# dspcraft/dsc

Measured on AMD Instinct MI355X. Metric: batched 1-D rfft GSamples/s, higher is better.
Workload: dtype f32

## Files before the change

### dsc_amd/csrc/fft_driver.cpp

```cpp
#include "dsc_internal.h"
#include "kernels.h"

#include <cmath>
#include <cstdlib>
#include <cstring>
#include <vector>

static void unit_root(long long k, long long n, long double *c, long double *s) {
    k %= n;
    const long long q = (4 * k) / n;
    const long long r = 4 * k - q * n;
    const long double a = 1.57079632679489661923132169163975144L * (long double) r / (long double) n;
    const long double cr = r == 0 ? 1.0L : cosl(a), sr = r == 0 ? 0.0L : sinl(a);
    switch (q) {
        case 0:  *c = cr;  *s = -sr; break;
        case 1:  *c = -sr; *s = -cr; break;
        case 2:  *c = -cr; *s = sr;  break;
        default: *c = sr;  *s = cr;  break;
    }
}

template<typename T>
static void fill_roots(T *dst, long long count, long long n) {
    for (long long k = 0; k < count; ++k) {
// ... 420 lines not shown
            ctx->last_fft_path = "regs_tiny";
            return;
        }
    }

    static const bool regs_mid_off = getenv("DSC_NO_REGS_MID") != nullptr;
    if (inner == 1 && !regs_mid_off && dsc_fft_regs_small_supports(j.L)) {
        const int x_n = j.x->shape[j.slot];
        const int want = j.mode == DSC_MODE_R2C_PACKED ? 2 * j.L : j.mode == DSC_MODE_C2R_PACKED ? j.L + 1 : j.L;
        const bool full = j.in_len == want && x_n == want;
        if (full || (long long) x_n * 16 * 256 < (1LL << 30)) {
            dsc_launch_fft_regs_mid(j.x->data, j.out->data, n_lines, j.L, j.mode, j.inverse, sp, plan->tw_full, plan->tw_real, j.scale,
                                    full ? -1 : x_n, j.in_len, ctx->stream);
            ctx->last_fft_path = "regs_small";
            return;
        }
    }
    if (inner == 1 && !regs_mid_off && dsc_fft_regs_mid_supports(j.L, j.mode, sp)) {
        const int x_n = j.x->shape[j.slot];
        const int want = j.mode == DSC_MODE_R2C_PACKED ? 2 * j.L : j.mode == DSC_MODE_C2R_PACKED ? j.L + 1 : j.L;
        const bool full = j.in_len == want && x_n == want;
        if (full || (long long) x_n * 16 * 64 < (1LL << 30)) {
            dsc_launch_fft_regs_mid(j.x->data, j.out->data, n_lines, j.L, j.mode, j.inverse, sp, plan->tw_full, plan->tw_real, j.scale,
                                    full ? -1 : x_n, j.in_len, ctx->stream);
            ctx->last_fft_path = "regs_mid";
            return;
        }
    }

    if (j.L <= dsc_fft_lds_max_len(sp)) {
        dsc_fft_lines_args a;
        a.in = j.x->data; a.out = j.out->data;
        a.n_lines = n_lines; a.inner = inner;
        a.lin = lin; a.lout = lout;
        a.L = j.L; a.in_len = j.in_len; a.inverse = j.inverse; a.scale = j.scale;
        a.tw = plan->tw_full; a.tw_real = plan->tw_real; a.tw4_len = 0; a.tw4 = nullptr;
        dsc_launch_fft_lines(a, j.mode, sp, ctx->stream);
        ctx->last_fft_path = "generic_lds";
        return;
    }
    run_four_step(ctx, j, sp, plan);
}

static dsc_tensor *make_out(dsc_ctx *ctx, const dsc_tensor *x, dsc_tensor *out, const int *out_shape, dsc_dtype out_dtype) {
    if (out == nullptr)
        return dsc_new_tensor(ctx, x->n_dim, &out_shape[DSC_MAX_DIMS - x->n_dim], out_dtype, nullptr);
    DSC_ASSERT(out->dtype == out_dtype);
    DSC_ASSERT(out->n_dim == x->n_dim);
    DSC_ASSERT(memcmp(out_shape, out->shape, DSC_MAX_DIMS * sizeof(int)) == 0);
    return out;
}

static dsc_tensor *internal_fft(dsc_ctx *ctx, const dsc_tensor *x, dsc_tensor *out, int n, int axis, bool forward) {
    DSC_ASSERT(x != nullptr);
    dsc_trace_scope trace__(ctx, forward ? "dsc_fft" : "dsc_ifft", "op;fft", x, nullptr, n, axis);
    const int slot = dsc_axis_slot(x, axis);
    DSC_ASSERT(slot >= 0 && slot < DSC_MAX_DIMS);
    const int x_n = x->shape[slot];
    n = n > 0 ? dsc_pow2_n(n) : dsc_pow2_n(x_n);

    int out_shape[DSC_MAX_DIMS];
    for (int i = 0; i < DSC_MAX_DIMS; ++i) out_shape[i] = i != slot ? x->shape[i] : n;
    dsc_dtype out_dtype = x->dtype;
    if (x->dtype == DSC_F32) out_dtype = DSC_C32;
    else if (x->dtype == DSC_F64) out_dtype = DSC_C64;
    out = make_out(ctx, x, out, out_shape, out_dtype);

    fft_job j;
    j.x = x; j.out = out; j.slot = slot;
    j.in_len = x_n < n ? x_n : n;
    j.L = n;
    j.mode = dsc_is_complex(x->dtype) ? DSC_MODE_C2C : DSC_MODE_R2C_CAST;
    j.inverse = !forward;
    j.scale = forward ? 1.0 : 1.0 / (double) n;
    run_job(ctx, j);
    return out;
}

static dsc_tensor *internal_rfft(dsc_ctx *ctx, const dsc_tensor *x, dsc_tensor *out, int n, int axis, bool forward) {
    DSC_ASSERT(x != nullptr);
    dsc_trace_scope trace__(ctx, forward ? "dsc_rfft" : "dsc_irfft", "op;fft", x, nullptr, n, axis);
    const int slot = dsc_axis_slot(x, axis);
    DSC_ASSERT(slot >= 0 && slot < DSC_MAX_DIMS);
    const int x_n = x->shape[slot];

    int out_n, order;
    dsc_dtype out_dtype;
    if (forward) {
        order = (n > 0 ? dsc_pow2_n(n) : dsc_pow2_n(x_n)) >> 1;
        out_n = order + 1;
        if (x->dtype == DSC_F32) out_dtype = DSC_C32;
        else if (x->dtype == DSC_F64) out_dtype = DSC_C64;
        else DSC_LOG_FATAL("RFFT input must be real");
    } else {
        DSC_ASSERT((n > 0 ? n : x_n) > 1);
        order = n > 0 ? dsc_pow2_n(n - 1) : dsc_pow2_n(x_n - 1);
        out_n = order << 1;
        if (x->dtype == DSC_C32) out_dtype = DSC_F32;
        else if (x->dtype == DSC_C64) out_dtype = DSC_F64;
        else DSC_LOG_FATAL("IRFFT input must be complex");
    }
    DSC_ASSERT(order >= 1);

    int out_shape[DSC_MAX_DIMS];
    for (int i = 0; i < DSC_MAX_DIMS; ++i) out_shape[i] = i != slot ? x->shape[i] : out_n;
    out = make_out(ctx, x, out, out_shape, out_dtype);

    fft_job j;
    j.x = x; j.out = out; j.slot = slot;
    j.L = order;
    j.inverse = !forward;
    if (forward) {
        j.mode = DSC_MODE_R2C_PACKED;
        j.in_len = x_n < 2 * order ? x_n : 2 * order;
        j.scale = 1.0;
    } else {
        j.mode = DSC_MODE_C2R_PACKED;
        j.in_len = x_n < order + 1 ? x_n : order + 1;
        j.scale = 2.0 / (double) (order << 1);
    }
    run_job(ctx, j);
    return out;
}

extern "C" dsc_tensor *dsc_fft(dsc_ctx *ctx, const dsc_tensor *x, dsc_tensor *out, int n, int axis) {
    return internal_fft(ctx, x, out, n, axis, true);
}
extern "C" dsc_tensor *dsc_ifft(dsc_ctx *ctx, const dsc_tensor *x, dsc_tensor *out, int n, int axis) {
    return internal_fft(ctx, x, out, n, axis, false);
}
extern "C" dsc_tensor *dsc_rfft(dsc_ctx *ctx, const dsc_tensor *x, dsc_tensor *out, int n, int axis) {
    return internal_rfft(ctx, x, out, n, axis, true);
}
extern "C" dsc_tensor *dsc_irfft(dsc_ctx *ctx, const dsc_tensor *x, dsc_tensor *out, int n, int axis) {
    return internal_rfft(ctx, x, out, n, axis, false);
}

extern "C" dsc_tensor *dsc_filter_fft(dsc_ctx *ctx, const dsc_tensor *s, const dsc_tensor *H, dsc_tensor *out) {
    DSC_ASSERT(s != nullptr && H != nullptr);
    DSC_TRACE_OP(ctx, "op;fft", s, H);
    DSC_ASSERT(dsc_is_complex(H->dtype));
    const int bins = H->shape[DSC_MAX_DIMS - 1];
    DSC_ASSERT(H->ne == bins && bins >= 2);
    const int n = 2 * (bins - 1);
    DSC_ASSERT((n & (n - 1)) == 0);

    const int ls = s->shape[DSC_MAX_DIMS - 1];
    if (s->dtype == DSC_F32 && H->dtype == DSC_C32 && n == 65536) {
        int out_shape[DSC_MAX_DIMS];
        memcpy(out_shape, s->shape, sizeof(out_shape));
        out_shape[DSC_MAX_DIMS - 1] = n;
        out = make_out(ctx, s, out, out_shape, DSC_F32);
        const dsc_fft_plan *plan = dsc_plan_fft(ctx, 32768, DSC_FFT_REAL, DSC_C32);
        dsc_launch_filter64k((const float *) s->data, H->data, (float *) out->data, s->ne / ls, ls, ls < n ? ls : n, plan->tw_aux, ctx->n_cu,
                             ctx->stream);
        ctx->last_fft_path = "filter_64k_regs";
        return out;
    }
    const bool sp_f = s->dtype == DSC_F32 && H->dtype == DSC_C32, dp_f = s->dtype == DSC_F64 && H->dtype == DSC_C64;
    if ((sp_f || dp_f) && dsc_fft_regs_mid_supports(n / 2, DSC_MODE_R2C_PACKED, sp_f) && n / 2 <= 16384 && (long long) ls * 8 * 64 < (1LL << 30)) {
        int out_shape[DSC_MAX_DIMS];
        memcpy(out_shape, s->shape, sizeof(out_shape));
        out_shape[DSC_MAX_DIMS - 1] = n;
        out = make_out(ctx, s, out, out_shape, s->dtype);
        const dsc_fft_plan *plan = dsc_plan_fft(ctx, n / 2, DSC_FFT_REAL, s->dtype);
        dsc_launch_filter_regs_mid(s->data, H->data, out->data, s->ne / ls, n / 2, sp_f, plan->tw_full, plan->tw_real, ls, ls < n ? ls : n,
                                   ctx->stream);
        ctx->last_fft_path = "filter_mid_regs";
        return out;
    }
    dsc_tensor *S = dsc_rfft(ctx, s, nullptr, n, -1);
    dsc_tensor *P = dsc_mul(ctx, S, const_cast<dsc_tensor *>(H), nullptr);
    out = dsc_irfft(ctx, P, out, -1, -1);
    dsc_tensor_free(ctx, S);
    dsc_tensor_free(ctx, P);
    ctx->last_fft_path = "filter_composed";
    return out;
}
```

### dsc_amd/csrc/fft_r2c_64k.hip

```cpp
#include "kernels.h"

#include <hip/hip_runtime.h>

#include <cmath>
#include <cstdlib>
#include <utility>

namespace {

typedef float f2 __attribute__((ext_vector_type(2)));

struct cf { float x, y; };
__device__ __forceinline__ cf operator+(cf a, cf b) { return cf{a.x + b.x, a.y + b.y}; }
__device__ __forceinline__ cf operator-(cf a, cf b) { return cf{a.x - b.x, a.y - b.y}; }
__device__ __forceinline__ cf to_cf(f2 a) { return cf{a.x, a.y}; }
__device__ __forceinline__ f2 to_f2(cf a) { return f2{a.x, a.y}; }

constexpr int kM = 32768;
constexpr int kRowPitch = 34;
constexpr int kPlaneFloats = 1024 * kRowPitch;
constexpr int kLdsBytes = kPlaneFloats * 4 + 1024 * 8;
constexpr int kTabEntries = 1024;

constexpr int kAuxW1024 = 0, kAuxW32768 = 1024, kAuxW65536 = 2048, kAuxEntries = 3072;
// ... 69 lines not shown
    dif_stage<INV, 2>(v, std::make_integer_sequence<int, 16>{});
}


#else
constexpr double kCos64d[17] = {
    1.0, 0.99518472667219688624, 0.98078528040323044913, 0.95694033573220886494,
    0.92387953251128675613, 0.88192126434835502971, 0.83146961230254523708, 0.77301045336273696081,
    0.70710678118654752440, 0.63439328416364549822, 0.55557023301960222474, 0.47139673682599764856,
    0.38268343236508977173, 0.29028467725446236764, 0.19509032201612826785, 0.09801714032956060199,
    0.0};

template<bool INV, int E>
__device__ __forceinline__ void dit_butterfly(cf &a, cf &b) {
    if constexpr (E == 0) {
        const cf u = a + b, d = a - b;
        a = u; b = d;
    } else if constexpr (E == 8) {
        const cf u = INV ? cf{a.x - b.y, a.y + b.x} : cf{a.x + b.y, a.y - b.x};
        const cf d = INV ? cf{a.x + b.y, a.y - b.x} : cf{a.x - b.y, a.y + b.x};
        a = u; b = d;
    } else {
        constexpr double c = E <= 8 ? kCos64d[2 * E] : -kCos64d[32 - 2 * E];
        constexpr double sn = (E <= 8 ? kCos64d[16 - 2 * E] : kCos64d[2 * E - 16]);
        constexpr double s = INV ? sn : -sn;
        if constexpr ((c < 0 ? -c : c) >= sn) {
            constexpr float t = (float) (s / c), cc = (float) c;
            float p, q;
            if constexpr (t == 1.0f) { p = b.x - b.y; q = b.y + b.x; }
            else if constexpr (t == -1.0f) { p = b.x + b.y; q = b.y - b.x; }
            else { p = __builtin_fmaf(-t, b.y, b.x); q = __builtin_fmaf(t, b.x, b.y); }
            const cf u = cf{__builtin_fmaf(cc, p, a.x), __builtin_fmaf(cc, q, a.y)};
            const cf d = cf{__builtin_fmaf(-cc, p, a.x), __builtin_fmaf(-cc, q, a.y)};
            a = u; b = d;
        } else {
            constexpr float r = (float) (c / s), ss = (float) s;
            const float pn = __builtin_fmaf(-r, b.x, b.y);
            const float q = __builtin_fmaf(r, b.y, b.x);
            const cf u = cf{__builtin_fmaf(-ss, pn, a.x), __builtin_fmaf(ss, q, a.y)};
            const cf d = cf{__builtin_fmaf(ss, pn, a.x), __builtin_fmaf(-ss, q, a.y)};
            a = u; b = d;
        }
    }
}

constexpr int brev_bits(int x, int bits) {
    int r = 0;
    for (int i = 0; i < bits; ++i) r |= ((x >> i) & 1) << (bits - 1 - i);
    return r;
}

template<bool INV, int S, int G, int... J>
__device__ __forceinline__ void dit_group(cf (&v)[32], std::integer_sequence<int, J...>) {
    constexpr int H = 32 >> S;
    constexpr int E = brev_bits(G, S - 1) * (16 >> (S - 1));
    (dit_butterfly<INV, E>(v[2 * H * G + J], v[2 * H * G + J + H]), ...);
}

template<bool INV, int S, int... G>
__device__ __forceinline__ void dit_stage(cf (&v)[32], std::integer_sequence<int, G...>) {
    (dit_group<INV, S, G>(v, std::make_integer_sequence<int, (32 >> S)>{}), ...);
}

template<bool INV>
__device__ __forceinline__ void dft32(cf (&v)[32]) {
    dit_stage<INV, 1>(v, std::make_integer_sequence<int, 1>{});
    dit_stage<INV, 2>(v, std::make_integer_sequence<int, 2>{});
    dit_stage<INV, 3>(v, std::make_integer_sequence<int, 4>{});
    dit_stage<INV, 4>(v, std::make_integer_sequence<int, 8>{});
    dit_stage<INV, 5>(v, std::make_integer_sequence<int, 16>{});
}
#endif

typedef unsigned int u2 __attribute__((ext_vector_type(2)));
typedef unsigned int u4 __attribute__((ext_vector_type(4)));
typedef float f4 __attribute__((ext_vector_type(4)));

template<int COMP>
__device__ __forceinline__ void plane_write(float *plane, int wbase, const cf (&v)[32]) {
    int wbase_hi = wbase + 16 * (32 * kRowPitch);
    asm("" : "+v"(wbase_hi));
    float *lo16 = plane + wbase;
    float *hi16 = plane + wbase_hi;
#pragma unroll
    for (int p = 0; p < 32; p += 2) lo16[br5(p) * (32 * kRowPitch)] = COMP == 0 ? v[p].x : v[p].y;
#pragma unroll
    for (int p = 1; p < 32; p += 2) hi16[(br5(p) - 16) * (32 * kRowPitch)] = COMP == 0 ? v[p].x : v[p].y;
}

#ifndef DSC_LDS_SPLIT_READS
#define DSC_LDS_SPLIT_READS 1
#endif
__device__ __forceinline__ f2 lds_read_b64(const f2 *p) {
#if DSC_LDS_SPLIT_READS
    return *(const volatile __attribute__((address_space(3))) f2 *) p;
#else
    return *p;
#endif
}

template<int COMP>
__device__ __forceinline__ void plane_read(const float *plane, int row, cf (&v)[32]) {
    const f2 *r = (const f2 *) (plane + __mul24(row, kRowPitch));
#pragma unroll
    for (int m = 0; m < 16; ++m) {
        const f2 t = lds_read_b64(r + m);
        if (COMP == 0) { v[2 * m].x = t.x; v[2 * m + 1].x = t.y; }
        else           { v[2 * m].y = t.x; v[2 * m + 1].y = t.y; }
    }
}

__device__ __forceinline__ void lds_barrier() {
    __builtin_amdgcn_fence(__ATOMIC_RELEASE, "workgroup", "local");
    __builtin_amdgcn_s_barrier();
    __builtin_amdgcn_fence(__ATOMIC_ACQUIRE, "workgroup", "local");
}

__device__ __forceinline__ float bperm(int byte_addr, float x) {
    return __int_as_float(__builtin_amdgcn_ds_bpermute(byte_addr, __float_as_int(x)));
}

__device__ __forceinline__ int column_of(int wave, int lane) {
    int kp = lane < 32 ? 32 * wave + lane : 1024 - 32 * wave - (63 - lane);
    return kp == 1024 ? 512 : kp;
}

#ifdef DSC_R2C64K_PROBE
#define PROBE_ARGS , int io_on
#define PROBE_NULL , 1
#define IO_ON io_on
#else
#define PROBE_ARGS
#define PROBE_NULL
#define IO_ON 1
#endif

__device__ __forceinline__ int thread_id(int wave_sgpr) {
    int zero;
    asm volatile("v_mov_b32 %0, 0" : "=v"(zero));
    const int lane = __builtin_amdgcn_mbcnt_hi(-1, __builtin_amdgcn_mbcnt_lo(-1, zero));
    return (wave_sgpr << 6) | lane;
}

#ifndef DSC_STREAM_AUX
#define DSC_STREAM_AUX 2
#endif
constexpr int kStream = DSC_STREAM_AUX;
__device__ __forceinline__ cf load_c(__amdgpu_buffer_rsrc_t r, int voff, int soff) {
    return to_cf(__builtin_bit_cast(f2, __builtin_amdgcn_raw_buffer_load_b64(r, voff, soff, kStream)));
}
#ifndef DSC_FILTER_EARLY_LOADS
#define DSC_FILTER_EARLY_LOADS 4
#endif
#ifndef DSC_IRFFT_PIN_PASS3
#define DSC_IRFFT_PIN_PASS3 1
#endif
#ifndef DSC_IRFFT_EARLY_PAIRS
#define DSC_IRFFT_EARLY_PAIRS 4
#endif
#ifndef DSC_IRFFT_LOAD_AUX
#define DSC_IRFFT_LOAD_AUX 0
#endif
__device__ __forceinline__ cf load_c_spec(__amdgpu_buffer_rsrc_t r, int voff, int soff) {
    return to_cf(__builtin_bit_cast(f2, __builtin_amdgcn_raw_buffer_load_b64(r, voff, soff, DSC_IRFFT_LOAD_AUX)));
}
__device__ __forceinline__ cf load_c_cached(__amdgpu_buffer_rsrc_t r, int voff, int soff) {
    return to_cf(__builtin_bit_cast(f2, __builtin_amdgcn_raw_buffer_load_b64(r, voff, soff, 0)));
}
template<int POLICY>
__device__ __forceinline__ void store_c(cf a, __amdgpu_buffer_rsrc_t r, int voff, int soff) {
    __builtin_amdgcn_raw_buffer_store_b64(__builtin_bit_cast(u2, to_f2(a)), r, voff, soff, POLICY);
}

__device__ __forceinline__ void fill_twiddle_table(f2 *T, const f2 *aux) {
    const int t = threadIdx.x;
    T[t] = aux[kAuxW1024 + (t >> 5) * (t & 31)];
    __syncthreads();
}

__device__ __forceinline__ void exchange(float *plane, int wbase, int row, const cf (&src)[32], cf (&dst)[32]) {
    plane_write<0>(plane, wbase, src);
    lds_barrier();
    plane_read<0>(plane, row, dst);
    lds_barrier();
    plane_write<1>(plane, wbase, src);
    lds_barrier();
    plane_read<1>(plane, row, dst);
    lds_barrier();
}

struct no_hook { __device__ __forceinline__ void operator()() const {} };

template<bool INV, typename Hook = no_hook>
__device__ __forceinline__ void three_passes(cf (&v)[32], float *plane, const f2 *T, const f2 *aux, int wave_sgpr,
                                             bool mirrored_in, bool mirrored_out, Hook before_pass3 = Hook{}) {
    dft32<INV>(v);
    cf u[32];
    {
        const int t = thread_id(wave_sgpr);
        const int col = mirrored_in ? column_of(t >> 6, t & 63) : t;
        const int hi = col >> 5;
        const f2 *th = T + hi;
#pragma unroll
        for (int r1 = 1; r1 < 32; ++r1) {
            const cf w = to_cf(th[32 * r1]);
            v[br5(r1)] = INV ? cmul_conj(v[br5(r1)], w) : cmul(v[br5(r1)], w);
        }
        exchange(plane, __mul24(col & 31, kRowPitch) + hi, t, v, u);
    }
    dft32<INV>(u);
    {
        const int t = thread_id(wave_sgpr);
        const int hi = t >> 5, lo = t & 31;
        const cf tw2_base = to_cf(aux[kAuxW32768 + __mul24(hi, lo)]);
        u[0] = INV ? cmul_conj(u[0], tw2_base) : cmul(u[0], tw2_base);
        const f2 *tl = T + lo;
#pragma unroll
        for (int r2 = 1; r2 < 32; ++r2) {
            const cf w = cmul(tw2_base, to_cf(tl[32 * r2]));
            u[br5(r2)] = INV ? cmul_conj(u[br5(r2)], w) : cmul(u[br5(r2)], w);
        }
        const int col_out = mirrored_out ? column_of(t >> 6, t & 63) : t;
        exchange(plane, __mul24(hi, kRowPitch) + lo, col_out, u, v);
    }
    before_pass3();
    dft32<INV>(v);
}

__device__ __forceinline__ void real_pair(cf p, cf q, cf wq, float hs, cf &out_k, cf &out_mk) {
    const cf s = cf{p.x + q.x, p.y - q.y};
    const cf d = cf{p.x - q.x, p.y + q.y};
    const cf wd = cmul(d, wq);
    out_k = cf{hs * s.x + wd.x, hs * s.y + wd.y};
    out_mk = cf{hs * s.x - wd.x, wd.y - hs * s.y};
}

__device__ __forceinline__ int partner_byte_addr(int wave, int lane) {
    return ((wave == 0 && (lane == 63 || lane == 0)) ? lane : 63 - lane) * 4;
}

#ifndef DSC_R2C64K_HELPERS_ONLY
__global__ __launch_bounds__(1024) void rfft64k_kernel(const float *__restrict__ x, f2 *__restrict__ X, int batch,
                                                       const f2 *__restrict__ aux, int in_pitch, int in_len PROBE_ARGS) {
    extern __shared__ __attribute__((aligned(16))) float lds[];
    float *plane = lds;
    f2 *T = (f2 *) (lds + kPlaneFloats);
    fill_twiddle_table(T, aux);

    const int wave_sgpr = __builtin_amdgcn_readfirstlane(threadIdx.x >> 6);

    cf v[32];
    {
        const int row0 = blockIdx.x;
        const __amdgpu_buffer_rsrc_t r0 = __builtin_amdgcn_make_buffer_rsrc(
            (void *) (x + (size_t) row0 * in_pitch), 0, row0 < batch ? in_len * 4 * IO_ON : 0, 0x00020000);
        const int load_off = thread_id(wave_sgpr) * 8;
#pragma unroll
        for (int j1 = 0; j1 < 32; ++j1) v[j1] = load_c(r0, load_off, j1 * 8192);
    }

    for (int row = blockIdx.x; row < batch; row += gridDim.x) {
        const int next_row = row + gridDim.x;
        const __amdgpu_buffer_rsrc_t rnext = __builtin_amdgcn_make_buffer_rsrc(
            (void *) (x + (size_t) next_row * in_pitch), 0, next_row < batch ? in_len * 4 * IO_ON : 0, 0x00020000);
        const __amdgpu_buffer_rsrc_t rout =
            __builtin_amdgcn_make_buffer_rsrc((void *) (X + (size_t) row * (kM + 1)), 0, (kM + 1) * 8 * IO_ON, 0x00020000);

        three_passes<false>(v, plane, T, aux, wave_sgpr, false, true);

        const int t4 = thread_id(wave_sgpr);
        const int lane = t4 & 63, wave = t4 >> 6;
        const int kp = column_of(wave, lane);
        const int partner_addr = partner_byte_addr(wave, lane);
        cf xk[16], xm[16];
        const cf zmid = v[br5(16)];
        if (wave_sgpr == 0) {
#pragma unroll
            for (int r = 16; r < 31; ++r) v[br5(r)] = lane == 0 ? v[br5(r + 1)] : v[br5(r)];
            v[br5(31)] = lane == 0 ? v[br5(0)] : v[br5(31)];
        }
#pragma unroll
        for (int k3 = 0; k3 < 16; ++k3) {
            const int src = 31 - br5(k3);
            xm[k3].x = bperm(partner_addr, v[src].x);
            xm[k3].y = bperm(partner_addr, v[src].y);
        }
        {
            const cf wpost = to_cf(aux[kAuxW65536 + kp]);
            const cf post_base = cf{0.5f * wpost.y, -0.5f * wpost.x};
#pragma unroll
            for (int k3 = 0; k3 < 16; ++k3) {
                const cf c = cf{root64_re(k3), root64_im(k3)};
                const cf w = k3 == 0 ? post_base : cmul(post_base, c);
                real_pair(v[br5(k3)], xm[k3], w, 0.5f, xk[k3], xm[k3]);
            }
        }

        f2 *stage = (f2 *) plane;
        const int skew = (int) ((((size_t) (X + (size_t) row * (kM + 1))) >> 3) & 15);
#pragma unroll
        for (int k3 = 0; k3 < 16; ++k3) stage[kp + 1024 * k3] = to_f2(xk[k3]);
        const cf xk15 = xk[15];
        const int load_off = thread_id(wave_sgpr) * 8;
#pragma unroll
        for (int j1 = 0; j1 < 16; ++j1) v[j1] = load_c(rnext, load_off, j1 * 8192);
        lds_barrier();
// ... 57 lines not shown
            real_pair(v[a], v[16 + a], wq, 0.5f * kScale, v[a], zm[i]);
        }
#pragma unroll
        for (int i = 0; i < 8; ++i) {
            const int a = half * 8 + i;
            v[16 + a].x = bperm(partner_addr, zm[i].x);
            v[16 + a].y = bperm(partner_addr, zm[i].y);
        }
    }
    cf w[32];
#pragma unroll
    for (int r = 0; r < 16; ++r) { w[r] = v[r]; w[16 + r] = v[31 - r]; }
    if (wave == 0) {
#pragma unroll
        for (int r = 31; r > 16; --r) w[r] = lane == 0 ? w[r - 1] : w[r];
        w[16] = lane == 0 ? cf{kScale * y_mid.x, -kScale * y_mid.y} : w[16];
    }
#pragma unroll
    for (int r = 0; r < 32; ++r) v[r] = w[r];
}

template<typename IssueNext>
__device__ __forceinline__ void staged_time_store(cf (&v)[32], float *plane, __amdgpu_buffer_rsrc_t rout, int wave_sgpr,
                                                  IssueNext issue_next) {
    f2 *stage = (f2 *) plane;
    const int t4 = thread_id(wave_sgpr);
#pragma unroll
    for (int p = 0; p < 32; p += 2) stage[t4 + 1024 * br5(p)] = to_f2(v[p]);
    issue_next(true);
    lds_barrier();
#pragma unroll
    for (int m = 0; m < 8; ++m) {
        const int k = 2 * (t4 + 1024 * m);
        const f2 lo2 = lds_read_b64(stage + k), hi2 = lds_read_b64(stage + k + 1);
        const f4 q = f4{lo2.x, lo2.y, hi2.x, hi2.y};
        __builtin_amdgcn_raw_buffer_store_b128(__builtin_bit_cast(u4, q), rout, k * 8, 0, kStream);
        if (m & 1) __builtin_amdgcn_sched_barrier(0);
    }
    lds_barrier();
#pragma unroll
    for (int p = 1; p < 32; p += 2) stage[t4 + 1024 * (br5(p) - 16)] = to_f2(v[p]);
    issue_next(false);
    lds_barrier();
#pragma unroll
    for (int m = 0; m < 8; ++m) {
        const int k = 2 * (t4 + 1024 * m);
        const f2 lo2 = lds_read_b64(stage + k), hi2 = lds_read_b64(stage + k + 1);
        const f4 q = f4{lo2.x, lo2.y, hi2.x, hi2.y};
        __builtin_amdgcn_raw_buffer_store_b128(__builtin_bit_cast(u4, q), rout, (kM / 2 + k) * 8, 0, kStream);
        if (m & 1) __builtin_amdgcn_sched_barrier(0);
    }
    lds_barrier();
}

__device__ __forceinline__ void unzip_rows(cf (&v)[32]) {
    cf nxt[32];
#pragma unroll
    for (int a = 0; a < 16; ++a) { nxt[a] = v[2 * a]; nxt[16 + a] = v[2 * a + 1]; }
#pragma unroll
    for (int a = 0; a < 32; ++a) v[a] = nxt[a];
}

#ifndef DSC_R2C64K_HELPERS_ONLY
__global__ __launch_bounds__(1024) void irfft64k_kernel(const f2 *__restrict__ X, float *__restrict__ x, int batch,
                                                        const f2 *__restrict__ aux, int in_pitch, int in_len PROBE_ARGS) {
    extern __shared__ __attribute__((aligned(16))) float lds[];
    float *plane = lds;
    f2 *T = (f2 *) (lds + kPlaneFloats);
    fill_twiddle_table(T, aux);

    const int wave_sgpr = __builtin_amdgcn_readfirstlane(threadIdx.x >> 6);

    cf v[32];
    cf y_mid = cf{0.f, 0.f};
    {
        const int row0 = blockIdx.x;
        const __amdgpu_buffer_rsrc_t r0 = __builtin_amdgcn_make_buffer_rsrc(
            (void *) (X + (size_t) row0 * in_pitch), 0, row0 < batch ? in_len * 8 * IO_ON : 0, 0x00020000);
        const int t0 = thread_id(wave_sgpr);
        const int c = column_of(t0 >> 6, t0 & 63);
        const int pv = (kM - c - 15 * 1024) * 8;
#pragma unroll
        for (int a = 0; a < 16; ++a) {
            v[a] = load_c_spec(r0, c * 8, a * 8192);
            v[16 + a] = load_c_spec(r0, pv, (15 - a) * 8192);
        }
        if (c == 0) y_mid = load_c_spec(r0, (kM / 2) * 8, 0);
    }

    for (int row = blockIdx.x; row < batch; row += gridDim.x) {
        const int next_row = row + gridDim.x;
        const __amdgpu_buffer_rsrc_t rnext = __builtin_amdgcn_make_buffer_rsrc(
            (void *) (X + (size_t) next_row * in_pitch), 0, next_row < batch ? in_len * 8 * IO_ON : 0, 0x00020000);
        const __amdgpu_buffer_rsrc_t rout =
            __builtin_amdgcn_make_buffer_rsrc((void *) (x + (size_t) row * 65536), 0, 65536 * 4 * IO_ON, 0x00020000);

        inverse_prepass_direct(v, y_mid, aux, wave_sgpr);
        constexpr int kEarly = DSC_IRFFT_EARLY_PAIRS;
        cf early[kEarly > 0 ? 2 * kEarly : 1];
        three_passes<true>(v, plane, T, aux, wave_sgpr, true, false, [&]() {
            if constexpr (kEarly > 0) {
                const int t3 = thread_id(wave_sgpr);
                const int c3 = column_of(t3 >> 6, t3 & 63);
                const int pv3 = (kM - c3 - 15 * 1024) * 8;
#pragma unroll
                for (int a = 0; a < kEarly; ++a) {
                    early[2 * a] = load_c_spec(rnext, c3 * 8, a * 8192);
                    early[2 * a + 1] = load_c_spec(rnext, pv3, (15 - a) * 8192);
                }
            }
        });

#if DSC_IRFFT_PIN_PASS3
#pragma unroll
        for (int p = 0; p < 32; p += 8)
            asm volatile("" : "+v"(v[p].x), "+v"(v[p].y), "+v"(v[p + 1].x), "+v"(v[p + 1].y), "+v"(v[p + 2].x), "+v"(v[p + 2].y), "+v"(v[p + 3].x),
                         "+v"(v[p + 3].y), "+v"(v[p + 4].x), "+v"(v[p + 4].y), "+v"(v[p + 5].x), "+v"(v[p + 5].y), "+v"(v[p + 6].x), "+v"(v[p + 6].y),
                         "+v"(v[p + 7].x), "+v"(v[p + 7].y));
#endif
        const int t4 = thread_id(wave_sgpr);
        const int c = column_of(t4 >> 6, t4 & 63);
        const int pv = (kM - c - 15 * 1024) * 8;
        staged_time_store(v, plane, rout, wave_sgpr, [&](bool first_half) {
            if (first_half) {
                y_mid = cf{0.f, 0.f};
                if (c == 0) y_mid = load_c_spec(rnext, (kM / 2) * 8, 0);
#pragma unroll
                for (int i = 0; i < 8; ++i) {
                    v[2 * i] = load_c_spec(rnext, c * 8, (kEarly + i) * 8192);
                    v[16 + 2 * i] = load_c_spec(rnext, pv, (15 - kEarly - i) * 8192);
                }
            } else {
#pragma unroll
                for (int i = 0; i < 8 - kEarly; ++i) {
                    v[2 * i + 1] = load_c_spec(rnext, c * 8, (kEarly + 8 + i) * 8192);
                    v[17 + 2 * i] = load_c_spec(rnext, pv, (7 - kEarly - i) * 8192);
                }
            }
        });
        {
            cf nxt[32];
#pragma unroll
            for (int a = 0; a < 16; ++a) {
                if (a < kEarly)          { nxt[a] = early[2 * a];             nxt[16 + a] = early[2 * a + 1]; }
                else if (a < kEarly + 8) { nxt[a] = v[2 * (a - kEarly)];      nxt[16 + a] = v[16 + 2 * (a - kEarly)]; }
                else                     { nxt[a] = v[2 * (a - kEarly - 8) + 1]; nxt[16 + a] = v[17 + 2 * (a - kEarly - 8)]; }
            }
#pragma unroll
            for (int a = 0; a < 32; ++a) v[a] = nxt[a];
        }
    }
}

__global__ __launch_bounds__(1024) void filter64k_kernel(const float *__restrict__ x, const f2 *__restrict__ H,
                                                         float *__restrict__ y, int batch, const f2 *__restrict__ aux, int in_pitch,
                                                         int in_len) {
    extern __shared__ __attribute__((aligned(16))) float lds[];
    float *plane = lds;
    f2 *T = (f2 *) (lds + kPlaneFloats);
    fill_twiddle_table(T, aux);

    const int wave_sgpr = __builtin_amdgcn_readfirstlane(threadIdx.x >> 6);
    const __amdgpu_buffer_rsrc_t rh = __builtin_amdgcn_make_buffer_rsrc((void *) H, 0, (kM + 1) * 8, 0x00020000);
    constexpr float kScale = 1.0f / (float) kM;

    cf v[32];
    {
        const int row0 = blockIdx.x;
        const __amdgpu_buffer_rsrc_t r0 = __builtin_amdgcn_make_buffer_rsrc(
            (void *) (x + (size_t) row0 * in_pitch), 0, row0 < batch ? in_len * 4 : 0, 0x00020000);
        const int load_off = thread_id(wave_sgpr) * 8;
#pragma unroll
        for (int j1 = 0; j1 < 32; ++j1) v[j1] = load_c(r0, load_off, j1 * 8192);
    }
    for (int row = blockIdx.x; row < batch; row += gridDim.x) {
        const int next_row = row + gridDim.x;
        const __amdgpu_buffer_rsrc_t rnext = __builtin_amdgcn_make_buffer_rsrc(
            (void *) (x + (size_t) next_row * in_pitch), 0, next_row < batch ? in_len * 4 : 0, 0x00020000);
        const __amdgpu_buffer_rsrc_t rout =
            __builtin_amdgcn_make_buffer_rsrc((void *) (y + (size_t) row * 65536), 0, 65536 * 4, 0x00020000);
        three_passes<false>(v, plane, T, aux, wave_sgpr, false, true);

        {
            const int t1 = thread_id(wave_sgpr);
            const int lane = t1 & 63, wave = t1 >> 6;
            const int c = column_of(wave, lane);
            const int partner_addr = partner_byte_addr(wave, lane);
            const cf wc = to_cf(aux[kAuxW65536 + c]);
            const cf post_base = cf{0.5f * wc.y, -0.5f * wc.x};
            const cf pre_base = cf{0.5f * kScale * wc.y, 0.5f * kScale * wc.x};
            if (wave == 0) {
                const cf zmid = v[br5(16)];
                const cf hmid = load_c_cached(rh, (kM / 2) * 8, 0);
                const cf pmid = cmul(cf{zmid.x, -zmid.y}, hmid);
                v[br5(16)] = lane == 0 ? cf{kScale * pmid.x, -kScale * pmid.y} : v[br5(16)];
            }
            cf park = v[br5(16)];
            if (wave == 0) {
#pragma unroll
                for (int r = 16; r < 31; ++r) v[br5(r)] = lane == 0 ? v[br5(r + 1)] : v[br5(r)];
                v[br5(31)] = lane == 0 ? v[br5(0)] : v[br5(31)];
            }
#pragma unroll
            for (int part = 0; part < 8; ++part) {
                cf q[2], zm[2];
#pragma unroll
                for (int i = 0; i < 2; ++i) {
                    const int a = part * 2 + i;
                    q[i].x = bperm(partner_addr, v[br5(31 - a)].x);
                    q[i].y = bperm(partner_addr, v[br5(31 - a)].y);
                }
#pragma unroll
                for (int i = 0; i < 2; ++i) {
                    const int a = part * 2 + i;
                    const cf w64 = cf{root64_re(a), root64_im(a)};
                    cf xk, xm;
                    real_pair(v[br5(a)], q[i], a == 0 ? post_base : cmul(post_base, w64), 0.5f, xk, xm);
                    const cf hk = load_c_cached(rh, c * 8, a * 8192);
                    const cf hm = load_c_cached(rh, (kM - 15 * 1024 - c) * 8, (15 - a) * 8192);
                    cf pk = cmul(xk, hk), pm = cmul(xm, hm);
                    if (a == 0) {
                        pk.y = (c == 0) ? 0.f : pk.y;
                        pm.y = (c == 0) ? 0.f : pm.y;
                    }
                    const cf w64c = cf{root64_re(a), -root64_im(a)};
                    real_pair(pk, pm, a == 0 ? pre_base : cmul(pre_base, w64c), 0.5f * kScale, v[br5(a)], zm[i]);
                }
#pragma unroll
                for (int i = 0; i < 2; ++i) {
                    const int a = part * 2 + i;
                    v[br5(31 - a)].x = bperm(partner_addr, zm[i].x);
                    v[br5(31 - a)].y = bperm(partner_addr, zm[i].y);
                }
                __builtin_amdgcn_sched_barrier(0);
            }
            if (wave == 0) {
#pragma unroll
                for (int r = 31; r > 16; --r) v[br5(r)] = lane == 0 ? v[br5(r - 1)] : v[br5(r)];
                v[br5(16)] = lane == 0 ? park : v[br5(16)];
            }
        }
        cf z[32];
#pragma unroll
        for (int r = 0; r < 32; ++r) z[r] = v[br5(r)];
        constexpr int kEarlyX = DSC_FILTER_EARLY_LOADS;
        cf early[kEarlyX > 0 ? kEarlyX : 1];
        three_passes<true>(z, plane, T, aux, wave_sgpr, true, false, [&]() {
            if constexpr (kEarlyX > 0) {
                const int off = thread_id(wave_sgpr) * 8;
#pragma unroll
                for (int j1 = 0; j1 < kEarlyX; ++j1) early[j1] = load_c(rnext, off, j1 * 8192);
            }
        });
        {
            const int load_off = thread_id(wave_sgpr) * 8;
            staged_time_store(z, plane, rout, wave_sgpr, [&](bool first_half) {
                if (first_half) {
#pragma unroll
                    for (int i = 0; i < 16; ++i) z[2 * i] = load_c(rnext, load_off, (kEarlyX + i) * 8192);
                } else {
#pragma unroll
                    for (int i = 0; i < 16 - kEarlyX; ++i) z[2 * i + 1] = load_c(rnext, load_off, (kEarlyX + 16 + i) * 8192);
                }
            });
#pragma unroll
            for (int j1 = 0; j1 < 32; ++j1) v[j1] = j1 < kEarlyX ? early[j1] : j1 < kEarlyX + 16 ? z[2 * (j1 - kEarlyX)] : z[2 * (j1 - kEarlyX - 16) + 1];
        }
    }
}

#endif

}

#ifndef DSC_R2C64K_HELPERS_ONLY
size_t dsc_r2c64k_table_bytes() { return (size_t) kAuxEntries * sizeof(float) * 2; }

void dsc_r2c64k_build_tables(void *host_dst) {
    float *o = (float *) host_dst;
    auto put = [&](int at, long long k, long long n) {
        const long double a = -2.0L * 3.14159265358979323846264338327950288L * (long double) k / (long double) n;
        o[2 * at] = (float) cosl(a);
        o[2 * at + 1] = (float) sinl(a);
    };
    for (int m = 0; m < kTabEntries; ++m) {
        put(kAuxW1024 + m, m, 1024);
        put(kAuxW32768 + m, m, 32768);
        put(kAuxW65536 + m, m, 65536);
    }
    o[2 * (kAuxW1024 + 256)] = 0.f;  o[2 * (kAuxW1024 + 256) + 1] = -1.f;
    o[2 * (kAuxW1024 + 512)] = -1.f; o[2 * (kAuxW1024 + 512) + 1] = 0.f;
    o[2 * (kAuxW1024 + 768)] = 0.f;  o[2 * (kAuxW1024 + 768) + 1] = 1.f;
}

void dsc_launch_rfft64k(const float *x, void *X, int batch, int in_pitch, int in_len, const void *aux, int n_cu, hipStream_t stream) {
    if (batch <= 0) return;
    static unsigned long long attr_devices = 0;
    if (dsc_first_use_on_device(attr_devices)) {
        DSC_KERNEL_CHECK(hipFuncSetAttribute((const void *) rfft64k_kernel, hipFuncAttributeMaxDynamicSharedMemorySize, kLdsBytes));
    }
    const int grid = batch < n_cu ? batch : n_cu;
    DSC_LAUNCH(rfft64k_kernel, dim3(grid), dim3(1024), kLdsBytes, stream, x, (f2 *) X, batch, (const f2 *) aux, in_pitch, in_len PROBE_NULL);
}

void dsc_launch_irfft64k(const void *X, float *x, int batch, int in_pitch, int in_len, const void *aux, int n_cu, hipStream_t stream) {
    if (batch <= 0) return;
    static unsigned long long attr_devices = 0;
    if (dsc_first_use_on_device(attr_devices)) {
        DSC_KERNEL_CHECK(hipFuncSetAttribute((const void *) irfft64k_kernel, hipFuncAttributeMaxDynamicSharedMemorySize, kLdsBytes));
    }
    const int grid = batch < n_cu ? batch : n_cu;
    DSC_LAUNCH(irfft64k_kernel, dim3(grid), dim3(1024), kLdsBytes, stream, (const f2 *) X, x, batch, (const f2 *) aux, in_pitch, in_len PROBE_NULL);
}
void dsc_launch_filter64k(const float *s, const void *H, float *y, int batch, int in_pitch, int in_len, const void *aux, int n_cu,
                          hipStream_t stream) {
    if (batch <= 0) return;
    static unsigned long long attr_devices = 0;
    if (dsc_first_use_on_device(attr_devices)) {
        DSC_KERNEL_CHECK(hipFuncSetAttribute((const void *) filter64k_kernel, hipFuncAttributeMaxDynamicSharedMemorySize, kLdsBytes));
    }
    const int grid = batch < n_cu ? batch : n_cu;
    DSC_LAUNCH(filter64k_kernel, dim3(grid), dim3(1024), kLdsBytes, stream, s, (const f2 *) H, y, batch, (const f2 *) aux, in_pitch, in_len);
}
#endif
```

### dsc_amd/csrc/kernels.h

```cpp
#pragma once

#include <hip/hip_runtime.h>
#include <cstddef>
#include <cstdio>
#include <cstdlib>

#define DSC_KERNEL_CHECK(call)                                                                                   \
    do {                                                                                                         \
        hipError_t kerr_ = (call);                                                                               \
        if (kerr_ != hipSuccess) {                                                                               \
            fprintf(stderr, "HIP error %s:%d: %s -> %s\n", __FILE__, __LINE__, #call, hipGetErrorString(kerr_)); \
            exit(EXIT_FAILURE);                                                                                  \
        }                                                                                                        \
    } while (0)
#define DSC_LAUNCH(...)                        \
    do {                                       \
        hipLaunchKernelGGL(__VA_ARGS__);       \
        DSC_KERNEL_CHECK(hipGetLastError());   \
    } while (0)

static inline bool dsc_first_use_on_device(unsigned long long &seen) {
    int dev = 0;
    DSC_KERNEL_CHECK(hipGetDevice(&dev));
    const unsigned long long bit = 1ull << (dev & 63);
    if (seen & bit) return false;
    seen |= bit;
    return true;
}

struct dsc_line_layout {
    long long outer_stride;
    long long inner_stride;
    long long elem_stride;
};

enum dsc_fft_mode {
    DSC_MODE_C2C = 0,
    DSC_MODE_R2C_CAST = 1,
    DSC_MODE_R2C_PACKED = 2,
    DSC_MODE_C2R_PACKED = 3,
};

struct dsc_fft_lines_args {
    const void *in;
    void *out;
    long long n_lines;
    long long inner;
    dsc_line_layout lin, lout;
    int L;
    int in_len;
    int inverse;
    double scale;
    const void *tw;
    const void *tw_real;
    long long tw4_len;
    const void *tw4;
};

int dsc_fft_lds_max_len(bool single_precision);

void dsc_launch_fft_lines(const dsc_fft_lines_args &a, dsc_fft_mode mode, bool single_precision, hipStream_t stream);

void dsc_launch_fft_pack(const void *in, void *work, long long q_first, long long n_lines, long long inner, dsc_line_layout lin,
                         int L, int in_len, dsc_fft_mode mode, bool single_precision, hipStream_t stream);
void dsc_launch_fft_c2r_prepass(const void *in, void *work, long long q_first, long long n_lines, long long inner, dsc_line_layout lin,
                                int L, int in_len, const void *tw_real, bool single_precision, hipStream_t stream);
void dsc_launch_fft_r2c_postpass(const void *work, void *out, long long q_first, long long n_lines, long long inner, dsc_line_layout lout,
                                 int L, const void *tw_real, bool single_precision, hipStream_t stream);
void dsc_launch_fft_unpack(const void *work, void *out, long long q_first, long long n_lines, long long inner, dsc_line_layout lout,
                           int L, double scale, dsc_fft_mode mode, bool single_precision, hipStream_t stream);

size_t dsc_r2c64k_table_bytes();
void   dsc_r2c64k_build_tables(void *host_dst);
void   dsc_launch_rfft64k(const float *x, void *X, int batch, int in_pitch, int in_len, const void *aux, int n_cu, hipStream_t stream);
void   dsc_launch_irfft64k(const void *X, float *x, int batch, int in_pitch, int in_len, const void *aux, int n_cu, hipStream_t stream);
void   dsc_launch_fft32k_c32(const void *z, void *Z, int batch, int in_pitch, int in_len, bool inverse, bool cast, const void *aux, int n_cu,
                             hipStream_t stream);
void   dsc_launch_filter64k(const float *s, const void *H, float *y, int batch, int in_pitch, int in_len, const void *aux, int n_cu,
                            hipStream_t stream);

bool   dsc_fft_regs_cols_supports(int L, dsc_fft_mode mode, bool single_precision);
void   dsc_launch_fft_regs_cols(const void *in, void *out, long long slices, int inner, int L, dsc_fft_mode mode, bool inverse, bool single_precision,
                                const void *tw_full, const void *tw_real, double scale, int in_axis, int in_len, int out_axis, hipStream_t stream);
bool   dsc_fft_cols_4step_split(int n, bool single_precision, int cols, int *n1, int *n2);
void   dsc_launch_rfft_cols_4step(const void *in, void *work, void *out, long long slices, int cc_n, int n1, int n2, bool single_precision,
                                  const void *tw1, const void *tw2, const void *twn, hipStream_t stream);
void   dsc_launch_irfft_cols_4step(const void *in, void *work, void *out, long long slices, int cc_n, int n1, int n2, bool single_precision,
                                   const void *tw1, const void *tw2, const void *twn, double scale, hipStream_t stream);
void   dsc_launch_fft_cols_4step(const void *in, void *work, void *out, long long slices, int inner, int n1, int n2, dsc_fft_mode mode, bool inverse,
                                 bool single_precision, const void *tw1, const void *tw2, const void *twn, double scale, hipStream_t stream);

bool   dsc_fft_two_pass_supports(int L, bool single_precision);
void   dsc_launch_fft_two_pass(const void *in, void *out, long long rows, int L, bool inverse, bool cast, bool single_precision, void *work,
                               const void *tw_full, long long in_pitch, int in_len, hipStream_t stream);
void   dsc_launch_rfft_two_pass(const void *in, void *out, long long rows, int L, bool inverse, bool single_precision, void *work,
                                const void *tw_full, const void *tw_real, long long in_pitch, int in_len, hipStream_t stream);

bool   dsc_fft_fused_l2_supports(int L, bool single_precision, bool real, bool inverse);
size_t dsc_fft_fused_l2_ctl_bytes();
size_t dsc_fft_fused_l2_scratch_bytes(int L, bool single_precision);
bool   dsc_launch_fft_fused_l2(const void *in, void *out, long long rows, int L, bool real, bool inverse, bool cast, bool single_precision, void *scratch,
                               unsigned *host_error, const void *tw_full, const void *tw_real, long long in_pitch, int in_len, hipStream_t stream);

bool dsc_fft_tiny_supports(int L);
void dsc_launch_fft_tiny_cols(const void *in, void *out, long long slices, int inner, int L, dsc_fft_mode mode, bool inverse, bool single_precision,
                              double scale, int in_axis, int in_len, int out_axis, hipStream_t stream);
void dsc_launch_fft_tiny(const void *in, void *out, long long n_lines, int L, dsc_fft_mode mode, bool inverse, bool single_precision, double scale,
                         long long in_pitch, int in_len, hipStream_t stream);

bool dsc_fft_regs_mid_supports(int L, dsc_fft_mode mode, bool single_precision);
bool dsc_fft_regs_small_supports(int L);
void dsc_launch_fft_regs_mid(const void *in, void *out, long long n_lines, int L, dsc_fft_mode mode, bool inverse, bool single_precision,
                             const void *tw_full, const void *tw_real, double scale, long long in_pitch, int in_len, hipStream_t stream);

void dsc_launch_filter_regs_mid(const void *s, const void *H, void *y, long long n_lines, int L, bool single_precision, const void *tw_full,
                                const void *tw_real, long long in_pitch, int in_len, hipStream_t stream);

bool dsc_stft_regs_supports(int n_fft);
void dsc_launch_stft_regs(const void *x, const void *w, void *out, long long n_lines, int n_fft, int T, int n_frames, int hop, int pad,
                          bool reflect, bool single_precision, int x_bytes, const void *tw_full, const void *tw_real, hipStream_t stream);
void dsc_launch_stft_frames(const void *x, const void *w, void *frames, long long q0, long long n_lines, int n_fft, long long T, int n_frames,
                            int hop, int pad, bool reflect, bool single_precision, hipStream_t stream);
void dsc_launch_istft_ola(const void *frames, const void *w, void *y, long long r0, long long rows, int fa, int fpr, int n_fft, int hop,
                          int n_frames, int pad, long long p0, long long p1, int length, bool single_precision, hipStream_t stream);

bool dsc_conv_regs_supports(int n);
void dsc_launch_conv_regs(const void *x, const void *H, void *y, long long n_lines, int n, int T, int n_blocks, int hop, int pad, int D, int T_out,
                          bool single_precision, int x_bytes, int y_bytes, const void *tw_full, const void *tw_real, hipStream_t stream);
void dsc_launch_conv_crop(const void *frames, void *y, long long q0, long long n_lines, int n, int D, int n_blocks, long long T_out,
                          bool single_precision, hipStream_t stream);
void dsc_launch_reverse(const void *in, void *out, int n, bool single_precision, hipStream_t stream);

bool dsc_hilbert_regs_supports(int n);
void dsc_launch_hilbert_regs(const void *x, void *out, long long n_lines, int n, bool envelope, bool single_precision, const void *tw_full,
                             const void *tw_real, long long in_pitch, int in_len, hipStream_t stream);
void dsc_launch_hilbert_response(void *H, int n, bool single_precision, hipStream_t stream);
void dsc_launch_hilbert_zip(const void *x, const void *y, void *out, long long q0, long long n_lines, int n, long long in_pitch, int in_len,
                            bool envelope, bool single_precision, bool y_double, hipStream_t stream);
void dsc_launch_hilbert_widen(const void *x, void *xw, long long q0, long long n_lines, long long in_pitch, int in_len, int wpitch,
                              hipStream_t stream);

bool dsc_fft2_regs_supports(int N0, int N1, dsc_fft_mode mode);
int dsc_fft2_regs_group(int N0, int N1, dsc_fft_mode mode, bool single_precision);
void dsc_launch_fft2_regs(const void *in, void *out, long long n_img, int N0, int N1, int h, int w, dsc_fft_mode mode, bool inverse,
                          bool single_precision, double scale, hipStream_t stream);

void dsc_launch_cast(const void *in, int in_dtype, void *out, int out_dtype, long long ne, hipStream_t stream);

void dsc_launch_unary(const void *in, int in_dtype, void *out, int op, long long ne, hipStream_t stream, double lo = 0, double hi = 0);
void dsc_launch_arange(void *out, int dtype, long long n, hipStream_t stream);

struct dsc_bcast_args {
    int out_shape[4];
    int a_stride[4];
    int b_stride[4];
    long long ne;
    int a_scalar, b_scalar;
    int fast;
    int small_ne;
};
void dsc_launch_binary(const void *a, const void *b, void *out, int dtype, int op, const dsc_bcast_args &g, hipStream_t stream);
bool dsc_launch_binary_mixed(const void *a, int a_dtype, const void *b, int b_dtype, void *out, int op, long long ne, hipStream_t stream);

void dsc_launch_reduce(const void *x, void *out, int dtype, int op, long long outer, int axis_n, long long inner,
                       void *workspace, size_t workspace_bytes, hipStream_t stream);

struct dsc_region {
    int count[4];
    long long stride[4];
    long long base;
    long long ne;
};
void dsc_launch_region_copy(const void *src, void *dst, int elem_bytes, const dsc_region &r, bool scatter, long long dense_ne,
                            hipStream_t stream);

void dsc_launch_transpose_last2(const void *in, void *out, int elem_bytes, long long batch, int rows, int cols, hipStream_t stream);
bool dsc_launch_transpose_moving_last(const void *in, void *out, int elem_bytes, int n_dim, const int *shape, const int *in_stride, const int *perm,
                                      hipStream_t stream);
```

Measured before the change: 652.1.

## Precompute two-term filter coefficients table to fuse r2c/c2r twiddles with H multiply

Adds a small kernel that folds the real-FFT split twiddles, the spectral filter H and the 1/N scale into a per-bin coefficient table (two complex coefficients per bin). The 64k fused filter kernel then loads this table with prefetching and applies the combined operation in a single partner-exchange pass, replacing the separate postpass/multiply/prepass arithmetic. This costs an extra launch and scratch memory per call, plus larger per-bin loads. It is gated by scratch capacity and an environment variable.

```diff
diff --git a/dsc_amd/csrc/fft_driver.cpp b/dsc_amd/csrc/fft_driver.cpp
--- a/dsc_amd/csrc/fft_driver.cpp
+++ b/dsc_amd/csrc/fft_driver.cpp
@@ -596,8 +596,14 @@
         out_shape[DSC_MAX_DIMS - 1] = n;
         out = make_out(ctx, s, out, out_shape, DSC_F32);
         const dsc_fft_plan *plan = dsc_plan_fft(ctx, 32768, DSC_FFT_REAL, DSC_C32);
-        dsc_launch_filter64k((const float *) s->data, H->data, (float *) out->data, s->ne / ls, ls, ls < n ? ls : n, plan->tw_aux, ctx->n_cu,
-                             ctx->stream);
+        const bool no_table = getenv("DSC_FILTER64K_NO_TABLE") != nullptr;
+        void *table = nullptr;
+        if (!no_table && ctx->scratch.capacity() >= dsc_filter64k_table_bytes() + DSC_DEVICE_ALIGN) {
+            ctx->scratch.reset();
+            table = ctx->scratch.alloc(dsc_filter64k_table_bytes());
+        }
+        dsc_launch_filter64k((const float *) s->data, H->data, (float *) out->data, s->ne / ls, ls, ls < n ? ls : n, plan->tw_aux, table,
+                             ctx->n_cu, ctx->stream);
         ctx->last_fft_path = "filter_64k_regs";
         return out;
     }
diff --git a/dsc_amd/csrc/fft_r2c_64k.hip b/dsc_amd/csrc/fft_r2c_64k.hip
--- a/dsc_amd/csrc/fft_r2c_64k.hip
+++ b/dsc_amd/csrc/fft_r2c_64k.hip
@@ -245,6 +245,15 @@
 #ifndef DSC_FILTER_EARLY_LOADS
 #define DSC_FILTER_EARLY_LOADS 4
 #endif
+#ifndef DSC_FILTER_TABLE_AHEAD
+#define DSC_FILTER_TABLE_AHEAD 2
+#endif
+#ifndef DSC_FILTER_TABLE_EARLY
+#define DSC_FILTER_TABLE_EARLY 1
+#endif
+#ifndef DSC_FILTER_TABLE_PIN_PASS3
+#define DSC_FILTER_TABLE_PIN_PASS3 1
+#endif
 #ifndef DSC_IRFFT_PIN_PASS3
 #define DSC_IRFFT_PIN_PASS3 1
 #endif
@@ -608,6 +617,36 @@
     }
 }
 
+constexpr int kCoeffThreads = 256;
+
+__global__ __launch_bounds__(kCoeffThreads) void two_term_coeff64k_kernel(const f2 *__restrict__ H, f4 *__restrict__ D) {
+    const int i = blockIdx.x * kCoeffThreads + threadIdx.x;
+    const int col = i & 1023, slot = i >> 10;
+    const int row = (col == 0 && slot >= 16) ? (slot == 31 ? 16 : slot + 1) : slot;
+    const int k = col + 1024 * row;
+    const f2 hk = H[k], hm = H[kM - k];
+    const double inv = 0.5 / (double) kM;
+    double d1r, d1i, d2r, d2i;
+    if (k == 0) {
+        d1r = (double) hk.x + (double) hm.x; d1i = 0.0;
+        d2r = 0.0;                           d2i = (double) hk.x - (double) hm.x;
+    } else {
+        double sn, cs;
+        sincospi((double) k / (double) kM, &sn, &cs);
+        const double er = (double) hk.x - (double) hm.x, ei = (double) hk.y + (double) hm.y;
+        d1r = (1.0 - sn) * (double) hk.x + (1.0 + sn) * (double) hm.x;
+        d1i = (1.0 - sn) * (double) hk.y - (1.0 + sn) * (double) hm.y;
+        d2r = -cs * ei;
+        d2i = cs * er;
+    }
+    D[i] = f4{(float) (d1r * inv), (float) (d1i * inv), (float) (d2r * inv), (float) (d2i * inv)};
+}
+
+__device__ __forceinline__ cf two_term(cf p, cf q, f4 d) {
+    return cf{d.x * p.x - d.y * p.y + d.z * q.x + d.w * q.y, d.x * p.y + d.y * p.x + d.w * q.x - d.z * q.y};
+}
+
+template<bool TABLE>
 __global__ __launch_bounds__(1024) void filter64k_kernel(const float *__restrict__ x, const f2 *__restrict__ H,
                                                          float *__restrict__ y, int batch, const f2 *__restrict__ aux, int in_pitch,
                                                          int in_len) {
@@ -617,7 +656,7 @@
     fill_twiddle_table(T, aux);
 
     const int wave_sgpr = __builtin_amdgcn_readfirstlane(threadIdx.x >> 6);
-    const __amdgpu_buffer_rsrc_t rh = __builtin_amdgcn_make_buffer_rsrc((void *) H, 0, (kM + 1) * 8, 0x00020000);
+    const __amdgpu_buffer_rsrc_t rh = __builtin_amdgcn_make_buffer_rsrc((void *) H, 0, TABLE ? kM * 16 : (kM + 1) * 8, 0x00020000);
     constexpr float kScale = 1.0f / (float) kM;
 
     cf v[32];
@@ -635,9 +674,72 @@
             (void *) (x + (size_t) next_row * in_pitch), 0, next_row < batch ? in_len * 4 : 0, 0x00020000);
         const __amdgpu_buffer_rsrc_t rout =
             __builtin_amdgcn_make_buffer_rsrc((void *) (y + (size_t) row * 65536), 0, 65536 * 4, 0x00020000);
-        three_passes<false>(v, plane, T, aux, wave_sgpr, false, true);
-
-        {
+        constexpr int kAhead = TABLE ? DSC_FILTER_TABLE_AHEAD : 0;
+        f4 dq[16][2];
+        auto table_offset = [&]() {
+            const int t0 = thread_id(wave_sgpr);
+            return column_of(t0 >> 6, t0 & 63) * 16;
+        };
+        auto load_d = [&](int part, int doff) {
+            dq[part][0] = __builtin_bit_cast(f4, __builtin_amdgcn_raw_buffer_load_b128(rh, doff, part * 16384, 0));
+            dq[part][1] = __builtin_bit_cast(f4, __builtin_amdgcn_raw_buffer_load_b128(rh, doff, (31 - part) * 16384, 0));
+        };
+        three_passes<false>(v, plane, T, aux, wave_sgpr, false, true, [&]() {
+            if constexpr (TABLE && DSC_FILTER_TABLE_EARLY) {
+                const int doff = table_offset();
+#pragma unroll
+                for (int part = 0; part < kAhead; ++part) load_d(part, doff);
+                __builtin_amdgcn_sched_barrier(0);
+            }
+        });
+
+        if constexpr (TABLE) {
+#if DSC_FILTER_TABLE_PIN_PASS3
+#pragma unroll
+            for (int p = 0; p < 32; p += 8)
+                asm volatile("" : "+v"(v[p].x), "+v"(v[p].y), "+v"(v[p + 1].x), "+v"(v[p + 1].y), "+v"(v[p + 2].x), "+v"(v[p + 2].y), "+v"(v[p + 3].x),
+                             "+v"(v[p + 3].y), "+v"(v[p + 4].x), "+v"(v[p + 4].y), "+v"(v[p + 5].x), "+v"(v[p + 5].y), "+v"(v[p + 6].x), "+v"(v[p + 6].y),
+                             "+v"(v[p + 7].x), "+v"(v[p + 7].y));
+#endif
+            const int t1 = thread_id(wave_sgpr);
+            const int lane = t1 & 63, wave = t1 >> 6;
+            const int partner_addr = partner_byte_addr(wave, lane);
+            if (wave_sgpr == 0) {
+                const cf r16 = v[br5(16)];
+#pragma unroll
+                for (int r = 16; r < 31; ++r) v[br5(r)] = lane == 0 ? v[br5(r + 1)] : v[br5(r)];
+                v[br5(31)] = lane == 0 ? r16 : v[br5(31)];
+            }
+            const int doff = table_offset();
+            if constexpr (!DSC_FILTER_TABLE_EARLY) {
+#pragma unroll
+                for (int part = 0; part < kAhead; ++part) load_d(part, doff);
+            }
+#pragma unroll
+            for (int part = 0; part < 16; ++part) {
+                const int sa = br5(part), sb = br5(31 - part);
+                if (part + kAhead < 16) load_d(part + kAhead, doff);
+                const f4 da = dq[part][0], db = dq[part][1];
+                const cf pa = v[sa], pb = v[sb];
+                cf send_a = pb, send_b = pa;
+                if (part == 0 && wave_sgpr == 0) {
+                    send_a = lane == 0 ? pa : pb;
+                    send_b = lane == 0 ? pb : pa;
+                }
+                const cf qa = cf{bperm(partner_addr, send_a.x), bperm(partner_addr, send_a.y)};
+                const cf qb = cf{bperm(partner_addr, send_b.x), bperm(partner_addr, send_b.y)};
+                v[sa] = two_term(pa, qa, da);
+                v[sb] = two_term(pb, qb, db);
+                asm volatile("" : "+v"(v[sa].x), "+v"(v[sa].y), "+v"(v[sb].x), "+v"(v[sb].y));
+                __builtin_amdgcn_sched_barrier(0);
+            }
+            if (wave_sgpr == 0) {
+                const cf r16 = v[br5(31)];
+#pragma unroll
+                for (int r = 31; r > 16; --r) v[br5(r)] = lane == 0 ? v[br5(r - 1)] : v[br5(r)];
+                v[br5(16)] = lane == 0 ? r16 : v[br5(16)];
+            }
+        } else {
             const int t1 = thread_id(wave_sgpr);
             const int lane = t1 & 63, wave = t1 >> 6;
             const int c = column_of(wave, lane);
@@ -768,14 +870,22 @@
     const int grid = batch < n_cu ? batch : n_cu;
     DSC_LAUNCH(irfft64k_kernel, dim3(grid), dim3(1024), kLdsBytes, stream, (const f2 *) X, x, batch, (const f2 *) aux, in_pitch, in_len PROBE_NULL);
 }
-void dsc_launch_filter64k(const float *s, const void *H, float *y, int batch, int in_pitch, int in_len, const void *aux, int n_cu,
-                          hipStream_t stream) {
+size_t dsc_filter64k_table_bytes() { return (size_t) kM * 16; }
+
+void dsc_launch_filter64k(const float *s, const void *H, float *y, int batch, int in_pitch, int in_len, const void *aux, void *table,
+                          int n_cu, hipStream_t stream) {
     if (batch <= 0) return;
     static unsigned long long attr_devices = 0;
     if (dsc_first_use_on_device(attr_devices)) {
-        DSC_KERNEL_CHECK(hipFuncSetAttribute((const void *) filter64k_kernel, hipFuncAttributeMaxDynamicSharedMemorySize, kLdsBytes));
+        DSC_KERNEL_CHECK(hipFuncSetAttribute((const void *) filter64k_kernel<true>, hipFuncAttributeMaxDynamicSharedMemorySize, kLdsBytes));
+        DSC_KERNEL_CHECK(hipFuncSetAttribute((const void *) filter64k_kernel<false>, hipFuncAttributeMaxDynamicSharedMemorySize, kLdsBytes));
     }
     const int grid = batch < n_cu ? batch : n_cu;
-    DSC_LAUNCH(filter64k_kernel, dim3(grid), dim3(1024), kLdsBytes, stream, s, (const f2 *) H, y, batch, (const f2 *) aux, in_pitch, in_len);
-}
-#endif
+    if (table != nullptr) {
+        DSC_LAUNCH(two_term_coeff64k_kernel, dim3(kM / kCoeffThreads), dim3(kCoeffThreads), 0, stream, (const f2 *) H, (f4 *) table);
+        DSC_LAUNCH(filter64k_kernel<true>, dim3(grid), dim3(1024), kLdsBytes, stream, s, (const f2 *) table, y, batch, (const f2 *) aux, in_pitch, in_len);
+    } else {
+        DSC_LAUNCH(filter64k_kernel<false>, dim3(grid), dim3(1024), kLdsBytes, stream, s, (const f2 *) H, y, batch, (const f2 *) aux, in_pitch, in_len);
+    }
+}
+#endif
diff --git a/dsc_amd/csrc/kernels.h b/dsc_amd/csrc/kernels.h
--- a/dsc_amd/csrc/kernels.h
+++ b/dsc_amd/csrc/kernels.h
@@ -76,8 +76,9 @@
 void   dsc_launch_irfft64k(const void *X, float *x, int batch, int in_pitch, int in_len, const void *aux, int n_cu, hipStream_t stream);
 void   dsc_launch_fft32k_c32(const void *z, void *Z, int batch, int in_pitch, int in_len, bool inverse, bool cast, const void *aux, int n_cu,
                              hipStream_t stream);
-void   dsc_launch_filter64k(const float *s, const void *H, float *y, int batch, int in_pitch, int in_len, const void *aux, int n_cu,
-                            hipStream_t stream);
+size_t dsc_filter64k_table_bytes();
+void   dsc_launch_filter64k(const float *s, const void *H, float *y, int batch, int in_pitch, int in_len, const void *aux, void *table,
+                            int n_cu, hipStream_t stream);
 
 bool   dsc_fft_regs_cols_supports(int L, dsc_fft_mode mode, bool single_precision);
 void   dsc_launch_fft_regs_cols(const void *in, void *out, long long slices, int inner, int L, dsc_fft_mode mode, bool inverse, bool single_precision,
```

Measured after the change: 634.7. -2.7%, worse.
